# PeterFWS/Structure-PLP-SLAM

Measured on AMD Instinct MI355X. Metric: frames/sec ORB+LSD extract+match, 640x480 TUM-RGBD, 1/2/4/8 GPU, higher is better.
Workload: dtype u8

## Files before the change

### structure-plp-slam_amd/csrc/line_context.hip

```cpp
#include <hip/hip_runtime.h>

#include <algorithm>
#include <cmath>
#include <cstring>
#include <mutex>
#include <vector>

#include "line_device.hpp"
#include "null4.hpp"
#include "seed_sort_model.hpp"
#include "sincos_ziv.hpp"
#include "plp_common.hpp"

using namespace plp;

struct plp_line {
    HostPinned pin;
    int device = 0;
    hipStream_t stream = nullptr;
    hipStream_t idle_stream = nullptr;
    int rows = 0, cols = 0, capB = 0;
    int grow_waves = 0;
    int seed_order = PLP_SEED_ORDER_LIBSTDCXX;
    bool mw_ok = false, seed_sort_ok = false;
    int mw_capB = 0, seed_capB = 0;
    LinePlanes P{};
    LsdParams lp{};
    ResizeExactTab rt{};
    BlurTapsN t11{}, t5{};
    LbdWeightsDev w{};
    DevBuf tabs, blur11, scaled, pix, g2, maxgrad, undef, order, n_order, reg, mw_heap, seed_ent, seed_ws, raw, n_raw, dx, dy, all_kl, all_kl_dir, all_lbd, n_all, status, prof, grow_stats;
    DevBuf l0copy, s_kl, s_lbd, s_fn, s_cnt;
    DevBuf aligned;
    int s_cap = 0;
    int last_B = 0;
    bool last_profiled = false;
    hipStream_t last_stream = nullptr;
    bool profiling = false;
    bool grow_big_ok = false;
    hipEvent_t ev[9] = {};
    double stage_ms[9] = {0, 0, 0, 0, 0, 0, 0, 0, 0};
    long stage_batches = 0;
    std::mutex mu;
};

namespace {

void gaussian_taps(int n, double sigma, int* out) {
    std::vector<double> k(n);
    double sum = 0;
    for (int i = 0; i < n; ++i) { const double x = i - (n - 1) * 0.5; k[i] = std::exp(-0.5 / (sigma * sigma) * x * x); sum += k[i]; }
    double err = 0;
    int acc = 0;
    for (int i = 0; i < n / 2; ++i) {
        const double adj = k[i] / sum * 256.0 + err;
        const int v = (int)std::nearbyint(adj);
        err = adj - v;
        out[i] = out[n - 1 - i] = v;
        acc += v;
    }
    out[n / 2] = 256 - 2 * acc;
}

int floor_d(double v) { int i = (int)v; return i - (i > v); }

void exact_coeffs(int ssize, int dsize, std::vector<int16_t>& ofs, std::vector<int16_t>& c1) {
    const double scale = 1.0 / ((double)dsize / ssize);
    for (int d = 0; d < dsize; ++d) {
        const double val = ((double)d + 0.5) * scale - 0.5;
        const int iv = floor_d(val);
        if (iv >= 0 && ssize > 1) {
            if (iv < ssize - 1) { ofs.push_back((int16_t)iv); c1.push_back((int16_t)std::nearbyint((val - (double)iv) * 256.0)); }
            else { ofs.push_back((int16_t)(ssize - 1)); c1.push_back(-1); }
        } else { ofs.push_back(0); c1.push_back(-2); }
    }
}

plp_status build(plp_line* c, int rows, int cols) {
    if (c->rows == rows && c->cols == cols) return PLP_OK;
    if (rows < 16 || cols < 16 || rows > 16000 || cols > 16000) return set_error(PLP_ERR_INVALID_ARG, "unsupported frame size for the line front-end");
    LinePlanes& P = c->P;
    P.W = cols; P.H = rows;
    P.sw = (int)std::nearbyint(cols * 0.5); P.sh = (int)std::nearbyint(rows * 0.5);
    P.sw_magic = (P.sw >= 2 && P.sw <= 8192) ? (uint32_t)(((1ull << 32) + (uint64_t)P.sw - 1) / (uint64_t)P.sw) : 0u;
// ... 7 lines not shown
    {
        uint32_t g = 0;
        while (g < 600000u && std::sqrt((double)g / 4.0) <= lp.rho) ++g;
        lp.g2_def_min = g;
    }
    lp.density_th = 0.6; lp.scale = 0.5; lp.n_bins = 1024; lp.refine = 1;
    const double LOG_NT = 5 * (std::log10((double)P.sw) + std::log10((double)P.sh)) / 2 + std::log10(11.0);
    lp.min_reg_size = (int)(size_t)(-LOG_NT / std::log10(lp.p));
    lp.min_length = (float)(0.125 * std::min(cols, rows));
    lp.keep_length = 60.f;
    const double sigma = 0.6 / 0.5;
    const unsigned h = (unsigned)std::ceil(sigma * std::sqrt(2 * 3.0 * std::log(10.0)));
    if (h != 5) return set_error(PLP_ERR_UNSUPPORTED, "unexpected LSD kernel size");
    gaussian_taps(11, sigma, c->t11.k);
    for (int i = 0; i < 11; ++i) c->t5.k[i] = 0;
    gaussian_taps(5, 1.0, c->t5.k);
    {
        double u = (7 * 3 - 1) / 2, sg = (7 * 2 + 1) / 2, inv = -1 / (2 * sg * sg);
        for (int i = 0; i < 21; ++i) { const double d = i - u; c->w.l[i] = (float)std::exp(d * d * inv); }
        u = (9 * 7 - 1) / 2; sg = u; inv = -1 / (2 * sg * sg);
        for (int i = 0; i < 63; ++i) { const double d = i - u; c->w.g[i] = (float)std::exp(d * d * inv); }
    }
    std::vector<int16_t> xo, xc, yo, yc;
    exact_coeffs(cols, P.sw, xo, xc);
    exact_coeffs(rows, P.sh, yo, yc);
    {
        bool plain = cols == 2 * P.sw && rows == 2 * P.sh;
        for (int i = 0; plain && i < P.sw; ++i) plain = xo[i] == 2 * i && xc[i] == 128;
        for (int i = 0; plain && i < P.sh; ++i) plain = yo[i] == 2 * i && yc[i] == 128;
        P.half_exact = plain ? 1 : 0;
    }
    std::vector<int16_t> blob;
    blob.insert(blob.end(), xo.begin(), xo.end()); blob.insert(blob.end(), xc.begin(), xc.end());
    blob.insert(blob.end(), yo.begin(), yo.end()); blob.insert(blob.end(), yc.begin(), yc.end());
    PLP_HIP(c->tabs.upload(blob.data(), blob.size() * 2, c->stream));
    PLP_HIP(hipStreamSynchronize(c->stream));
    const int16_t* base = (const int16_t*)c->tabs.p;
    c->rt.xo = base; c->rt.xc = base + P.sw; c->rt.yo = base + 2 * P.sw; c->rt.yc = base + 2 * P.sw + P.sh;
    c->rows = rows; c->cols = cols; c->capB = 0; c->mw_capB = 0; c->seed_capB = 0;
    return PLP_OK;
}

plp_status ensure(plp_line* c, int B) {
    LinePlanes& P = c->P;
    const size_t n = (size_t)P.sw * P.sh, nv = (size_t)(P.sw - 1) * (P.sh - 1);
    const int Bmw = std::min(B, kLsdMwMaxFrames);
    if (B > c->capB) {
        if (!P.half_exact) PLP_HIP(c->blur11.reserve((size_t)P.pitch * P.H * B));
        PLP_HIP(c->scaled.reserve((size_t)P.spitch * P.sh * B));
        PLP_HIP(c->pix.reserve(n * sizeof(LsdPix) * B));
        PLP_HIP(c->g2.reserve(n * 4 * B)); PLP_HIP(c->n_order.reserve(4 * (size_t)B)); PLP_HIP(c->maxgrad.reserve(4 * ((n + 255) / 256) * (size_t)B)); PLP_HIP(c->undef.reserve((n + 63) / 64 * 8 * B));
        PLP_HIP(c->order.reserve(nv * 4 * B)); PLP_HIP(c->reg.reserve(std::max(n * (size_t)B, 2 * n * (size_t)Bmw) * 4));
        PLP_HIP(c->raw.reserve(sizeof(float4) * kLineCap * B)); PLP_HIP(c->n_raw.reserve(4 * (size_t)B));
        PLP_HIP(c->dx.reserve(dxy_frame_entries(P.W, P.H) * 4 * B));
        PLP_HIP(c->all_kl.reserve(sizeof(plp_keyline) * kLineCap * B)); PLP_HIP(c->all_kl_dir.reserve(sizeof(float2) * kLineCap * B)); PLP_HIP(c->all_lbd.reserve((size_t)32 * kLineCap * B));
        PLP_HIP(c->n_all.reserve(4 * (size_t)B)); PLP_HIP(c->status.reserve(16)); PLP_HIP(c->prof.reserve(128)); PLP_HIP(c->grow_stats.reserve(16 * (size_t)B));
        P.blur11 = (uint8_t*)c->blur11.p; P.scaled = (uint8_t*)c->scaled.p;
        P.pix = (LsdPix*)c->pix.p; P.g2 = (uint32_t*)c->g2.p; P.n_order = (int32_t*)c->n_order.p;
        P.blockmax = (uint32_t*)c->maxgrad.p; P.undef = (unsigned long long*)c->undef.p;
        P.order = (uint32_t*)c->order.p; P.reg = (uint32_t*)c->reg.p; P.raw = (float4*)c->raw.p; P.n_raw = (int32_t*)c->n_raw.p;
        P.dxy = (short2*)c->dx.p; P.all_kl = (plp_keyline*)c->all_kl.p; P.all_kl_dir = (float2*)c->all_kl_dir.p; P.all_lbd = (uint8_t*)c->all_lbd.p;
        P.n_all = (int32_t*)c->n_all.p; P.status = (int32_t*)c->status.p; P.prof = (long long*)c->prof.p; P.grow_stats = (int32_t*)c->grow_stats.p;
        c->capB = B;
    }
    P.reg_frame_stride = B <= kLsdMwMaxFrames ? 2 * n : n;
    P.mw_heap_frame_stride = (size_t)(kMwMaxWaves - 1) * kMwHeapBufs * kMwHeap;
    if (c->mw_ok && B <= kLsdMwMaxFrames && B > c->mw_capB) {
        PLP_HIP(c->mw_heap.reserve(P.mw_heap_frame_stride * 4 * (size_t)B));
        c->mw_capB = B;
    }
    P.mw_heap = (B <= c->mw_capB) ? (uint32_t*)c->mw_heap.p : nullptr;
    if (c->seed_order == PLP_SEED_ORDER_LIBSTDCXX && B > c->seed_capB) {
        PLP_HIP(c->seed_ent.reserve(nv * 4 * (size_t)B)); PLP_HIP(c->seed_ws.reserve(seed_sort_ws_entries(nv) * 4 * (size_t)B));
        c->seed_capB = B;
    }
    return PLP_OK;
}

plp_status run(plp_line* c, const uint8_t* d_imgs, int B, int rows, int cols, size_t step, size_t frame_stride, plp_keyline* d_kl,
               uint8_t* d_lbd, double* d_fn, int cap, int32_t* d_counts, hipStream_t st) {
    PLP_HIP(hipSetDevice(c->device));
    if (c->seed_order == PLP_SEED_ORDER_LIBSTDCXX && !c->seed_sort_ok)
        return set_error(PLP_ERR_UNSUPPORTED, "this device refused the dynamic LDS size of the exact seed sort (144 KB per workgroup): select PLP_SEED_ORDER_STABLE with plp_line_set_seed_order");
    PLP_TRY(build(c, rows, cols));
    PLP_TRY(ensure(c, B));
    if (((uintptr_t)d_imgs % 4 == 0) && (step % 4 == 0) && (frame_stride % 4 == 0)) {
        c->P.img = d_imgs; c->P.img_frame_stride = frame_stride; c->P.img_pitch = (int)step;
    } else {
        const size_t fs = (size_t)c->P.pitch * rows;
        PLP_HIP(c->aligned.reserve(fs * B));
        for (int f = 0; f < B; ++f)
            PLP_HIP(hipMemcpy2DAsync((uint8_t*)c->aligned.p + f * fs, c->P.pitch, d_imgs + f * frame_stride, step, cols, rows, hipMemcpyDeviceToDevice, st));
        c->P.img = (const uint8_t*)c->aligned.p; c->P.img_frame_stride = fs; c->P.img_pitch = c->P.pitch;
    }
    PLP_HIP(hipMemsetAsync(c->status.p, 0, 16, st));
    if (c->profiling) PLP_HIP(hipMemsetAsync(c->prof.p, 0, 128, st));
    const bool exact = c->seed_order == PLP_SEED_ORDER_LIBSTDCXX;
    c->lp.seed_exact = exact ? 1 : 0;
    const SeedSortBufs ssb{(uint32_t*)c->seed_ent.p, (uint32_t*)c->seed_ws.p, seed_sort_ws_entries((size_t)(c->P.sw - 1) * (c->P.sh - 1))};
    launch_line_front(st, c->P, c->lp, c->rt, c->t11, c->t5, c->w, d_kl, d_lbd, d_fn, cap, d_counts, B, c->profiling ? c->ev : nullptr,
                      c->grow_waves, exact ? &ssb : nullptr, c->mw_ok);
    PLP_HIP(hipGetLastError());
    if (c->profiling) {
        PLP_HIP(hipEventSynchronize(c->ev[8]));
        for (int i = 0; i < 8; ++i) { float ms = 0; PLP_HIP(hipEventElapsedTime(&ms, c->ev[i], c->ev[i + 1])); c->stage_ms[i] += ms; }
        float tot = 0; PLP_HIP(hipEventElapsedTime(&tot, c->ev[0], c->ev[8])); c->stage_ms[8] += tot;
        ++c->stage_batches;
    }
    c->last_B = B; c->last_stream = st; c->last_profiled = c->profiling;
    return PLP_OK;
}

plp_status batch_status(const int32_t s[4], bool check_cap) {
    if (check_cap && (s[0] & 1)) return set_error(PLP_ERR_CAPACITY, "a frame produced more lines than `cap`; output truncated");
// ... 166 lines not shown
    for (int i = 0; i < 9; ++i) ms9[i] = c->stage_ms[i];
    if (n_batches) *n_batches = c->stage_batches;
    return PLP_OK;
}

plp_status plp_line_scaled_size(const plp_line* c, int32_t* rows, int32_t* cols) {
    if (!c || !rows || !cols || !c->rows) return set_error(PLP_ERR_INVALID_ARG, "no frame processed yet");
    *rows = c->P.sh; *cols = c->P.sw;
    return PLP_OK;
}

plp_status plp_line_debug_read(plp_line* c, plp_line_debug_id what, int32_t frame, void* dst, size_t dst_bytes, int64_t* n_out) {
    if (!c || !dst || !n_out) return set_error(PLP_ERR_INVALID_ARG, "NULL argument");
    std::lock_guard<std::mutex> lk(c->mu);
    if (!c->last_B || frame < 0 || frame >= c->last_B) return set_error(PLP_ERR_INVALID_ARG, "bad frame");
    PLP_HIP(hipSetDevice(c->device));
    PLP_HIP(hipStreamSynchronize(c->last_stream));
    const LinePlanes& P = c->P;
    const size_t n = (size_t)P.sw * P.sh, nv = (size_t)(P.sw - 1) * (P.sh - 1), full = (size_t)P.W * P.H;
    int32_t cnt = 0;
    switch (what) {
        case PLP_LINE_DBG_SCALED:
            if (dst_bytes < n) return set_error(PLP_ERR_CAPACITY, "dst too small");
            PLP_HIP(hipMemcpy2D(dst, P.sw, P.scaled + (size_t)frame * P.spitch * P.sh, P.spitch, P.sw, P.sh, hipMemcpyDeviceToHost));
            *n_out = (int64_t)n; return PLP_OK;
        case PLP_LINE_DBG_ORDER:
            PLP_HIP(hipMemcpy(&cnt, P.n_order + frame, 4, hipMemcpyDeviceToHost));
            if (dst_bytes < (size_t)cnt * 4) return set_error(PLP_ERR_CAPACITY, "dst too small");
            if (cnt) PLP_HIP(hipMemcpy(dst, P.order + (size_t)frame * nv, (size_t)cnt * 4, hipMemcpyDeviceToHost));
            *n_out = cnt; return PLP_OK;
        case PLP_LINE_DBG_RAW:
            PLP_HIP(hipMemcpy(&cnt, P.n_raw + frame, 4, hipMemcpyDeviceToHost));
            if (dst_bytes < (size_t)cnt * 16) return set_error(PLP_ERR_CAPACITY, "dst too small");
            if (cnt) PLP_HIP(hipMemcpy(dst, P.raw + (size_t)frame * kLineCap, (size_t)cnt * 16, hipMemcpyDeviceToHost));
            *n_out = cnt; return PLP_OK;
        case PLP_LINE_DBG_ALL_KL:
        case PLP_LINE_DBG_ALL_LBD: {
            PLP_HIP(hipMemcpy(&cnt, P.n_all + frame, 4, hipMemcpyDeviceToHost));
            const size_t rec = what == PLP_LINE_DBG_ALL_KL ? sizeof(plp_keyline) : 32;
            if (dst_bytes < (size_t)cnt * rec) return set_error(PLP_ERR_CAPACITY, "dst too small");
            const uint8_t* src = what == PLP_LINE_DBG_ALL_KL ? (const uint8_t*)(P.all_kl + (size_t)frame * kLineCap) : P.all_lbd + (size_t)frame * kLineCap * 32;
            if (cnt) PLP_HIP(hipMemcpy(dst, src, (size_t)cnt * rec, hipMemcpyDeviceToHost));
            *n_out = cnt; return PLP_OK;
        }
        case PLP_LINE_DBG_GROW_STATS:
            if (dst_bytes < 16) return set_error(PLP_ERR_CAPACITY, "dst too small");
            PLP_HIP(hipMemcpy(dst, P.grow_stats + (size_t)frame * 4, 16, hipMemcpyDeviceToHost));
            *n_out = 4; return PLP_OK;
        case PLP_LINE_DBG_SOBEL_DX:
        case PLP_LINE_DBG_SOBEL_DY:
            if (dst_bytes < full * 2) return set_error(PLP_ERR_CAPACITY, "dst too small");
            {
                const size_t ent = dxy_frame_entries(P.W, P.H);
                std::vector<int16_t> both(ent * 2);
                PLP_HIP(hipMemcpy(both.data(), P.dxy + (size_t)frame * ent, ent * 4, hipMemcpyDeviceToHost));
                int16_t* d16 = (int16_t*)dst;
                const int tiles8 = (P.W + 7) / 8;
                for (int y = 0; y < P.H; ++y)
                    for (int x = 0; x < P.W; ++x) d16[(size_t)y * P.W + x] = both[2 * (size_t)dxy_index(x, y, tiles8) + (what == PLP_LINE_DBG_SOBEL_DY ? 1 : 0)];
            }
            *n_out = (int64_t)full; return PLP_OK;
    }
    return set_error(PLP_ERR_INVALID_ARG, "unknown debug id");
}

int32_t plp_model_sincos_host(const float* a, int64_t n, float* c, float* s, uint8_t* proven) {
    int32_t n_proven = 0;
    for (int64_t i = 0; i < n; ++i) { proven[i] = plp::sincos_ziv(a[i], c + i, s + i) ? 1 : 0; n_proven += proven[i]; }
    return n_proven;
}

int32_t plp_model_null_vector4_host(const double* A, int32_t n, double* out_v, int32_t* out_sweeps) {
    if (!A || !out_v || n < 0) return -1;
    for (int32_t i = 0; i < n; ++i) {
        int sweeps = 0;
        plp::null_vector4(A + 16 * (size_t)i, out_v + 4 * (size_t)i, &sweeps);
        if (out_sweeps) out_sweeps[i] = sweeps;
    }
    return n;
}

int32_t plp_model_seed_introsort_host(uint32_t* entries, int64_t n, int32_t depth_limit, uint32_t skip_key) {
    if (!entries || n < 0 || n > (int64_t)kLsdMaxScaledPixels) return -1;
    plp::seedsort::introsort_loop_model(entries, (int)n, depth_limit, skip_key);
    return 0;
}

plp_status plp_seed_introsort_debug(int32_t device, uint32_t* entries, int64_t n, int32_t depth_limit, uint32_t skip_key, int32_t variant, int32_t* n_live) {
    if (!entries || n < 0 || n > (int64_t)kLsdMaxScaledPixels) return set_error(PLP_ERR_INVALID_ARG, "bad entries");
    int nd = 0;
    if (hipGetDeviceCount(&nd) != hipSuccess || nd == 0) return set_error(PLP_ERR_NO_DEVICE, "no HIP device visible");
    PLP_HIP(hipSetDevice(device));
    PLP_HIP(seed_sort_configure());
    if (depth_limit < 0) { int lg = 0; while ((2ll << lg) <= n) ++lg; depth_limit = 2 * lg; }
    DevBuf ent, ws, st;
    const int copies = std::max(1, std::min(4096, getenv("PLP_SEED_SORT_DBG_COPIES") ? atoi(getenv("PLP_SEED_SORT_DBG_COPIES")) : 1));
    PLP_HIP(ent.reserve((size_t)std::max<int64_t>(n, 1) * 4 * copies)); PLP_HIP(ws.reserve(seed_sort_ws_entries((size_t)n) * 4 * copies)); PLP_HIP(st.reserve(16));
    for (int k = 0; k < copies; ++k) PLP_HIP(hipMemcpy((uint32_t*)ent.p + (size_t)k * n, entries, (size_t)n * 4, hipMemcpyHostToDevice));
    PLP_HIP(hipMemset(st.p, 0, 16));
    DevBuf dbg;
    const char* dflag = getenv("PLP_SEED_SORT_DBG");
    if (dflag) { PLP_HIP(dbg.reserve(4 * (2 + 6 * 4000 + 48))); PLP_HIP(hipMemset(dbg.p, 0, 4 * (2 + 6 * 4000 + 48))); int f = atoi(dflag); PLP_HIP(hipMemcpy(dbg.p, &f, 4, hipMemcpyHostToDevice)); }
    launch_seed_sort_debug(nullptr, (uint32_t*)ent.p, (int)n, depth_limit, skip_key, (uint32_t*)ws.p, (int32_t*)st.p, dflag ? (int*)dbg.p : nullptr, variant, copies);
    PLP_HIP(hipGetLastError());
    PLP_HIP(hipDeviceSynchronize());
    int32_t s = 0;
    PLP_HIP(hipMemcpy(&s, st.p, 4, hipMemcpyDeviceToHost));
    PLP_HIP(hipMemcpy(entries, ent.p, (size_t)n * 4, hipMemcpyDeviceToHost));
// ... 12 lines not shown
```

### structure-plp-slam_amd/csrc/line_device.hpp

```cpp
#pragma once
#include <hip/hip_runtime.h>
#include <stdint.h>

#include "../../include/plp_front.h"

namespace plp {

constexpr int kMwHeap = 16384;
constexpr int kMwHeapBufs = 2;
constexpr int kMwMaxWaves = 8;
constexpr int kLsdMwMaxFrames = 256;
constexpr int kLineCap = 2048;
constexpr double kLsdNotDef = -1024.0;
constexpr int kLsdSeedPixBits = 20;
constexpr uint32_t kLsdSeedPixMask = (1u << kLsdSeedPixBits) - 1u;
constexpr size_t kLsdGrowLdsBytes = 66560;
constexpr size_t kLsdMaxScaledPixels = (kLsdGrowLdsBytes / 4 - 256) * 32 - 31;
static_assert(kLsdMaxScaledPixels <= (size_t)kLsdSeedPixMask + 1, "seed packing of k_lsd_order must hold every admitted pixel index");
static_assert(kLsdSeedPixBits + 10 <= 32, "10 bits of gradient bin above the pixel field");

struct alignas(16) LsdPix { float deg; uint32_t g2; float2 cs; };
__device__ __forceinline__ double pix_ang(const LsdPix& p) { return (double)p.deg * (3.14159265358979323846 / 180); }
__device__ __forceinline__ double pix_mod(const LsdPix& p) { return sqrt((double)p.g2 / 4.0); }

struct LinePlanes {
    int W, H;
    int sw, sh;
    uint32_t sw_magic;
    int pitch, spitch;
    const uint8_t* img; size_t img_frame_stride; int img_pitch;
    uint8_t* blur11;
    uint8_t* scaled;
    LsdPix* pix;
    uint32_t* g2;
    uint32_t* blockmax;
    unsigned long long* undef;
    uint32_t* order;
    int32_t* n_order;
    uint32_t* reg; size_t reg_frame_stride;
    uint32_t* mw_heap; size_t mw_heap_frame_stride;
    float4* raw; int32_t* n_raw;
    short2* dxy;
    plp_keyline* all_kl; uint8_t* all_lbd; int32_t* n_all;
    float2* all_kl_dir;
    int32_t* status;
    int half_exact;
    int32_t* grow_stats;
    long long* prof;
};

__host__ __device__ inline size_t dxy_frame_entries(int W, int H) { return (size_t)((W + 7) / 8) * ((H + 3) / 4) * 32; }
__host__ __device__ inline int dxy_index(int x, int y, int tiles_x) { return (((y >> 2) * tiles_x + (x >> 3)) << 5) + ((y & 3) << 3) + (x & 7); }

struct LsdParams {
    double prec, p, rho, density_th, scale;
    int n_bins, refine, min_reg_size;
    float min_length;
    float keep_length;
    float c_pass, c_fail;
    uint32_t g2_def_min;
    int seed_exact;
};
constexpr double kLsdAngleBand = 3.5e-4;
constexpr double kLsdBandMinPrec = 0.01, kLsdBandMaxPrec = 1.5;

struct ResizeExactTab { const int16_t *xo, *xc, *yo, *yc; };
struct BlurTapsN { int k[11]; };
struct LbdWeightsDev { float g[63], l[21]; };

struct SeedSortBufs { uint32_t* ent; uint32_t* ws; size_t ws_stride; };
size_t seed_sort_ws_entries(size_t nv);
hipError_t seed_sort_configure();
void launch_seed_order_exact(hipStream_t st, const LinePlanes& P, const LsdParams& lp, int B, uint32_t* ent, uint32_t* ws, size_t ws_stride);
void launch_seed_sort_debug(hipStream_t st, uint32_t* ent, int n, int depth, uint32_t skip_key, uint32_t* ws, int32_t* status, int* dbg, int variant, int copies = 1);
hipError_t grow_mw_configure();
hipError_t grow_configure();

void launch_line_front(hipStream_t st, const LinePlanes& P, const LsdParams& lp, const ResizeExactTab& rt, const BlurTapsN& t11,
                       const BlurTapsN& t5, const LbdWeightsDev& w, plp_keyline* out_kl, uint8_t* out_lbd, double* out_fn, int cap,
                       int32_t* out_counts, int B, hipEvent_t* ev, int grow_waves, const SeedSortBufs* seed_exact, bool mw_ok);

}
```

### structure-plp-slam_amd/csrc/line_kernels.hip

```cpp
#include <hip/hip_runtime.h>
#include <stdint.h>

#include <algorithm>
#include <cstdlib>

#include "blur_tile.hpp"
#include "plp_barrier.hpp"
#include "line_device.hpp"
#include "plp_common.hpp"
#include "sincos_ziv.hpp"
#include "xcd_map.hpp"

namespace plp {

struct TileDiv { uint32_t gx_magic, tiles_x_magic; };
static inline TileDiv tile_div(int tiles, int tiles_x, int B) { return TileDiv{plp_div_magic((uint32_t)tiles, (uint64_t)tiles * B), plp_div_magic((uint32_t)tiles_x, (uint64_t)tiles)}; }

__device__ __forceinline__ int reflect101_l(int p, int len) {
    if (len == 1) return 0;
    while (p < 0 || p >= len) p = p < 0 ? -p : 2 * (len - 1) - p;
    return p;
}

__device__ __forceinline__ float fast_atan2_deg_l(float y, float x) {
// ... 1369 lines not shown
        run += __popcll(bal);
    }
    if (lane == 0) P.n_all[b] = run;
}

constexpr int kSobelTW = 120, kSobelTH = 30;
static_assert(sizeof(BlurTileLds<2>::in) >= kBlurTH * (kBlurTW / 4) * 4, "the blurred tile must fit the input rows it replaces");
__global__ __launch_bounds__(256) __attribute__((amdgpu_waves_per_eu(8, 8))) void k_blur_sobel(const uint8_t* __restrict__ src, size_t src_fs, int src_pitch,
                                                                                            short2* __restrict__ dxy, int w, int h, BlurTapsN taps, TileDiv td) {
    __shared__ __attribute__((aligned(16))) BlurTileLds<2> Sb;
    uint32_t* const bt = reinterpret_cast<uint32_t*>(Sb.in);
    const int tiles_x = (w + kSobelTW - 1) / kSobelTW;
    unsigned t, f;
    xcd_frame_major(t, f, td.gx_magic);
    const int trow = (int)plp_div(t, (unsigned)tiles_x, td.tiles_x_magic);
    const int bx0 = ((int)t - trow * tiles_x) * kSobelTW - 4, by0 = trow * kSobelTH - 1;
    blur_tile_core<2>(Sb, src + (size_t)f * src_fs, src_pitch, w, h, bx0, by0, taps.k, [&](int r0, int c4, const uint32_t (&rows)[kBlurRS]) {
#pragma unroll
        for (int rr = 0; rr < kBlurRS; ++rr) bt[(r0 + rr) * (kBlurTW / 4) + c4 / 4] = rows[rr];
    });
    wg_barrier();
    short2* out_frame = dxy + (size_t)f * dxy_frame_entries(w, h);
    const int tiles8 = (w + 7) / 8;
    for (int i = threadIdx.x; i < (kSobelTW / 4) * (kSobelTH / 2); i += 256) {
        const int cgp = i % (kSobelTW / 4), rp = i / (kSobelTW / 4);
        const int x = bx0 + 4 + 4 * cgp, y = by0 + 1 + 2 * rp;
        if (x >= w || y >= h) continue;
        const int cd = 1 + cgp;
        int d[4][4], sm[4][4];
#pragma unroll
        for (int r = 0; r < 4; ++r) {
            const uint32_t* q = &bt[(2 * rp + r) * (kBlurTW / 4) + cd];
            const uint32_t A = q[-1], Bv = q[0], Cv = q[1];
            const int p[6] = {(int)(A >> 24), (int)(Bv & 255u), (int)((Bv >> 8) & 255u), (int)((Bv >> 16) & 255u), (int)(Bv >> 24), (int)(Cv & 255u)};
#pragma unroll
            for (int k = 0; k < 4; ++k) { d[r][k] = p[k + 2] - p[k]; sm[r][k] = p[k] + 2 * p[k + 1] + p[k + 2]; }
        }
#pragma unroll
        for (int j = 0; j < 2; ++j) {
            if (y + j >= h) continue;
            uint32_t out[4];
#pragma unroll
            for (int k = 0; k < 4; ++k)
                out[k] = ((uint32_t)(d[j][k] + 2 * d[j + 1][k] + d[j + 2][k]) & 0xffffu) | ((uint32_t)(sm[j + 2][k] - sm[j][k]) << 16);
            *reinterpret_cast<uint4*>(out_frame + dxy_index(x, y + j, tiles8)) = make_uint4(out[0], out[1], out[2], out[3]);
        }
    }
}

__constant__ int c_comb[32][2] = {{0, 1}, {0, 2}, {0, 3}, {0, 4}, {0, 5}, {0, 6}, {1, 2}, {1, 3}, {1, 4}, {1, 5}, {1, 6},
                                  {2, 3}, {2, 4}, {2, 5}, {2, 6}, {2, 7}, {2, 8}, {3, 4}, {3, 5}, {3, 6}, {3, 7}, {3, 8},
                                  {4, 5}, {4, 6}, {4, 7}, {4, 8}, {5, 6}, {5, 7}, {5, 8}, {6, 7}, {6, 8}, {7, 8}};

constexpr int kLbdU = 8;
__global__ __launch_bounds__(256) void k_lbd(LinePlanes P, LbdWeightsDev W) {
    __shared__ float s_row[4][63][8];
    __shared__ float s_des[4][72], s_des2[4][72], s_norm[4][4];
    const int lane = threadIdx.x & 63, wv = __builtin_amdgcn_readfirstlane((int)(threadIdx.x >> 6)), b = blockIdx.y;
    const int n_lines = P.n_all[b];
    for (int li = blockIdx.x * 4 + wv; li < n_lines; li += gridDim.x * 4) {
    const plp_keyline kl = P.all_kl[(size_t)b * kLineCap + li];
    const short2* dxyImg = P.dxy + (size_t)b * dxy_frame_entries(P.W, P.H);
    const int tiles8 = (P.W + 7) / 8;
    const short imageWidth = (short)(P.W - 1), imageHeight = (short)(P.H - 1);
    const short lengthOfLSP = (short)kl.numOfPixels;
    const short halfWidth = (short)((lengthOfLSP - 1) / 2), halfHeight = 31;
    const float midX = (float)(0.5 * (double)__fadd_rn(kl.sPointInOctaveX, kl.ePointInOctaveX));
    const float midY = (float)(0.5 * (double)__fadd_rn(kl.sPointInOctaveY, kl.ePointInOctaveY));
    const float2 dir = P.all_kl_dir[(size_t)b * kLineCap + li];
    const float dL0 = dir.x, dL1 = dir.y;
    const float dO0 = -dL1, dO1 = dL0;
    if (lane < 63) {
        float sCorX0 = __fadd_rn(__fadd_rn(__fmul_rn(-dL0, (float)halfWidth), __fmul_rn(dL1, (float)halfHeight)), midX);
        float sCorY0 = __fadd_rn(__fsub_rn(__fmul_rn(-dL1, (float)halfWidth), __fmul_rn(dL0, (float)halfHeight)), midY);
        for (int r = 0; r < lane; ++r) { sCorX0 = __fsub_rn(sCorX0, dL1); sCorY0 = __fadd_rn(sCorY0, dL0); }
        float sCorX = sCorX0, sCorY = sCorY0;
        float pgdL = 0, ngdL = 0, pgdO = 0, ngdO = 0;
        for (int w0 = 0; w0 < lengthOfLSP; w0 += kLbdU) {
            int off[kLbdU];
#pragma unroll
            for (int u = 0; u < kLbdU; ++u) {
                short t = (short)roundf(sCorX);
                const short xCor = (t < 0) ? 0 : (t > imageWidth) ? imageWidth : t;
                t = (short)roundf(sCorY);
                const short yCor = (t < 0) ? 0 : (t > imageHeight) ? imageHeight : t;
                off[u] = dxy_index(xCor, yCor, tiles8);
                sCorX = __fadd_rn(sCorX, dL0);
                sCorY = __fadd_rn(sCorY, dL1);
            }
            short2 vxy[kLbdU];
#pragma unroll
            for (int u = 0; u < kLbdU; ++u) vxy[u] = dxyImg[off[u]];
#pragma unroll
            for (int u = 0; u < kLbdU; ++u) {
                if (w0 + u < lengthOfLSP) {
                    const float fx = (float)vxy[u].x, fy = (float)vxy[u].y;
                    const float gDL = __fadd_rn(__fmul_rn(fx, dL0), __fmul_rn(fy, dL1));
                    const float gDO = __fadd_rn(__fmul_rn(fx, dO0), __fmul_rn(fy, dO1));
                    if (gDL > 0) pgdL = __fadd_rn(pgdL, gDL); else ngdL = __fsub_rn(ngdL, gDL);
                    if (gDO > 0) pgdO = __fadd_rn(pgdO, gDO); else ngdO = __fsub_rn(ngdO, gDO);
                }
            }
        }
        const float cg = W.g[lane];
        pgdL = __fmul_rn(cg, pgdL); ngdL = __fmul_rn(cg, ngdL); pgdO = __fmul_rn(cg, pgdO); ngdO = __fmul_rn(cg, ngdO);
        float* r = s_row[wv][lane];
        r[0] = pgdL; r[1] = ngdL; r[2] = __fmul_rn(pgdL, pgdL); r[3] = __fmul_rn(ngdL, ngdL);
        r[4] = pgdO; r[5] = ngdO; r[6] = __fmul_rn(pgdO, pgdO); r[7] = __fmul_rn(ngdO, ngdO);
    }
    __builtin_amdgcn_fence(__ATOMIC_RELEASE, "workgroup");
    __builtin_amdgcn_wave_barrier();
    for (int item = lane; item < 72; item += 64) {
        const int band = item >> 3, comp = item & 7;
        const bool sq = (comp == 2 || comp == 3 || comp == 6 || comp == 7);
        float acc = 0;
        for (int hID = max(0, (band - 1) * 7); hID < min(63, (band + 2) * 7); ++hID) {
            const int rb = hID / 7;
            const float c = rb == band ? W.l[hID % 7 + 7] : (rb == band + 1 ? W.l[hID % 7 + 14] : W.l[hID % 7]);
            const float v = s_row[wv][hID][comp];
            acc = sq ? __fadd_rn(acc, __fmul_rn(__fmul_rn(c, c), v)) : __fadd_rn(acc, __fmul_rn(c, v));
        }
        s_des[wv][item] = acc;
    }
    __builtin_amdgcn_fence(__ATOMIC_RELEASE, "workgroup");
    __builtin_amdgcn_wave_barrier();
    float* des = s_des2[wv];
    auto wave_sync = [] { __builtin_amdgcn_fence(__ATOMIC_ACQ_REL, "workgroup"); __builtin_amdgcn_wave_barrier(); };
    if (lane < 36) {
        const int band = lane >> 2, k = lane & 3;
        const float invN = (band == 0 || band == 8) ? (float)(1.0 / (7 * 2.0)) : (float)(1.0 / (7 * 3.0));
        const float* sb = &s_des[wv][band * 8];
        const int mi = (k < 2) ? k : k + 2, qi = mi + 2;
        const float temp = __fmul_rn(sb[mi], invN);
        des[band * 8 + k] = temp;
        des[band * 8 + 4 + k] = sqrtf(__fsub_rn(__fmul_rn(sb[qi], invN), __fmul_rn(temp, temp)));
    }
    wave_sync();
    if (lane == 0) {
        float tempM = 0, tempS = 0;
        for (int band = 0; band < 9; ++band) {
            const float* v = des + 8 * band;
            for (int k = 0; k < 4; ++k) tempM = __fadd_rn(tempM, __fmul_rn(v[k], v[k]));
            for (int k = 4; k < 8; ++k) tempS = __fadd_rn(tempS, __fmul_rn(v[k], v[k]));
        }
        s_norm[wv][0] = __fdiv_rn(1.0f, sqrtf(tempM));
        s_norm[wv][1] = __fdiv_rn(1.0f, sqrtf(tempS));
    }
    wave_sync();
    for (int i = lane; i < 72; i += 64) {
        float v = __fmul_rn(des[i], s_norm[wv][(i >> 2) & 1]);
        if ((double)v > 0.4) v = (float)0.4;
        des[i] = v;
    }
    wave_sync();
    if (lane == 0) {
        float temp = 0;
        for (int i = 0; i < 72; ++i) temp = __fadd_rn(temp, __fmul_rn(des[i], des[i]));
        s_norm[wv][2] = __fdiv_rn(1.0f, sqrtf(temp));
    }
    wave_sync();
    for (int i = lane; i < 72; i += 64) des[i] = __fmul_rn(des[i], s_norm[wv][2]);
    wave_sync();
    if (lane < 32) {
        const float* f1 = des + 8 * c_comb[lane][0];
        const float* f2 = des + 8 * c_comb[lane][1];
        unsigned r = 0;
        for (int i = 0; i < 8; ++i) r += (f1[i] > f2[i]) ? (1u << i) : 0u;
        P.all_lbd[((size_t)b * kLineCap + li) * 32 + lane] = (uint8_t)r;
    }
    __builtin_amdgcn_fence(__ATOMIC_ACQ_REL, "workgroup");
    __builtin_amdgcn_wave_barrier();
    }
}

__global__ __launch_bounds__(64) void k_line_finalize(LinePlanes P, LsdParams lp, plp_keyline* __restrict__ out_kl,
                                                      uint8_t* __restrict__ out_lbd, double* __restrict__ out_fn, int cap,
                                                      int32_t* __restrict__ out_counts) {
    const int b = blockIdx.x, lane = threadIdx.x;
    const int n = P.n_all[b];
    int run = 0;
    for (int base = 0; base < n; base += 64) {
        const int i = base + lane;
        plp_keyline kl{};
        bool keep = false;
        if (i < n) { kl = P.all_kl[(size_t)b * kLineCap + i]; keep = kl.octave == 0 && kl.lineLength >= lp.keep_length; }
        const unsigned long long bal = __ballot(keep);
        const int o = run + __popcll(bal & ((1ull << lane) - 1ull));
        if (keep && o < cap) {
            out_kl[(size_t)b * cap + o] = kl;
            const uint4* s = reinterpret_cast<const uint4*>(P.all_lbd + ((size_t)b * kLineCap + i) * 32);
            uint4* d = reinterpret_cast<uint4*>(out_lbd + ((size_t)b * cap + o) * 32);
            d[0] = s[0]; d[1] = s[1];
            const double sx = kl.startPointX, sy = kl.startPointY, ex = kl.endPointX, ey = kl.endPointY;
            const double a = sy * 1.0 - 1.0 * ey, bb = 1.0 * ex - sx * 1.0, c = sx * ey - sy * ex;
            const double nrm = sqrt(a * a + bb * bb);
            double* f = out_fn + ((size_t)b * cap + o) * 3;
            f[0] = a / nrm; f[1] = bb / nrm; f[2] = c / nrm;
        }
        run += __popcll(bal);
    }
    if (lane == 0) {
        out_counts[b] = min(run, cap);
        if (run > cap) atomicOr(P.status, 1);
    }
}

void launch_line_front(hipStream_t st, const LinePlanes& P, const LsdParams& lp, const ResizeExactTab& rt, const BlurTapsN& t11,
                       const BlurTapsN& t5, const LbdWeightsDev& w, plp_keyline* out_kl, uint8_t* out_lbd, double* out_fn, int cap,
                       int32_t* out_counts, int B, hipEvent_t* ev, int grow_waves, const SeedSortBufs* seed_exact, bool mw_ok) {
    auto mark = [&](int i) { if (ev) (void)hipEventRecord(ev[i], st); };
    const bool sobel_first = !ev;
    const size_t plane_fs = (size_t)P.pitch * P.H, splane_fs = (size_t)P.spitch * P.sh;
    const int tiles = ((P.W + 127) / 128) * ((P.H + kBlurTH - 1) / kBlurTH);
    const int sobel_tiles = ((P.W + kSobelTW - 1) / kSobelTW) * ((P.H + kSobelTH - 1) / kSobelTH);
    const TileDiv blur_td = tile_div(tiles, (P.W + 127) / 128, B), sobel_td = tile_div(sobel_tiles, (P.W + kSobelTW - 1) / kSobelTW, B);
    mark(0);
    if (sobel_first) hipLaunchKernelGGL(k_blur_sobel, dim3(sobel_tiles, B), dim3(256), 0, st, P.img, P.img_frame_stride, P.img_pitch, P.dxy, P.W, P.H, t5, sobel_td);
    if (P.half_exact)
        hipLaunchKernelGGL(k_blur_half, dim3(tiles, B), dim3(256), 0, st, P.img, P.img_frame_stride, P.img_pitch, P.scaled, splane_fs, P.spitch, P.W, P.H, t11, blur_td);
    else {
        hipLaunchKernelGGL(k_blur_plane<5>, dim3(tiles, B), dim3(256), 0, st, P.img, P.img_frame_stride, P.img_pitch, P.blur11, plane_fs,
                           P.pitch, P.W, P.H, t11, blur_td);
        hipLaunchKernelGGL(k_resize_exact, dim3((P.sw + 255) / 256, (P.sh + 3) / 4, B), dim3(64, 4), 0, st, P.blur11, plane_fs, P.pitch,
                           P.scaled, splane_fs, P.spitch, P.sw, P.sh, rt);
    }
    mark(1);
    const int n = P.sw * P.sh;
    hipLaunchKernelGGL(k_lsd_gradient, dim3((n + 255) / 256, B), dim3(256), 0, st, P, lp);
    mark(2);
    if (seed_exact) launch_seed_order_exact(st, P, lp, B, seed_exact->ent, seed_exact->ws, seed_exact->ws_stride);
    else hipLaunchKernelGGL(k_lsd_order, dim3(B), dim3(256), 0, st, P, lp, (n + 255) / 256);
    mark(3);
    constexpr int ring = 256;
    const size_t per_wave = (size_t)((((n + 31) / 32 + 1) & ~1) + ring) * 4;
    const int wpb = (int)std::max<size_t>(1, std::min<size_t>(4, 65536 / per_wave));
    MwLayout L{};
    size_t mw_bytes = 0;
    const int want_waves = grow_waves > 0 ? std::min(grow_waves, kMwMaxWaves) : kMwMaxWaves;
    if (mw_ok && B <= kLsdMwMaxFrames && want_waves >= 2 && P.mw_heap && P.reg_frame_stride >= 2 * (size_t)n) {
        const int nw_al = (((n + 31) / 32 + 1) & ~1), groups_cap = ((P.sw - 1) * (P.sh - 1) + kMwGroup - 1) / kMwGroup + 64 / kMwGroup;
        for (int w = want_waves; w >= 2; --w) {
            const size_t bytes = (size_t)5 * nw_al * 4 + (size_t)w * (nw_al + 256 + kMwAssumed + 2) * 4 + (8 + (4 + 2 * kMwBufs) * kMwMaxWaves) * 4 + ((groups_cap + 15) & ~15) + 16 +
                                 (size_t)(w - 1) * kMwBufs * kMwEntries * sizeof(MwEntry);
            if (bytes <= 160 * 1024) { L.waves = w; L.ring = 256; L.nw_al = nw_al; L.n_groups_cap = groups_cap; L.lookahead = kMwBufs * (w - 1); L.policy = 0; L.prof = ev ? 1 : 0; mw_bytes = bytes; break; }
        }
    }
    if (L.waves >= 2)
        hipLaunchKernelGGL(k_lsd_grow_mw, dim3(B), dim3(64 * L.waves), mw_bytes, st, P, lp, L);
    else
        hipLaunchKernelGGL(k_lsd_grow, dim3((B + wpb - 1) / wpb), dim3(64 * wpb), per_wave * wpb, st, P, lp, B, wpb, ring);
    mark(4);
    hipLaunchKernelGGL(k_keylines, dim3(B), dim3(64), 0, st, P, lp);
    mark(5);
    if (!sobel_first) hipLaunchKernelGGL(k_blur_sobel, dim3(sobel_tiles, B), dim3(256), 0, st, P.img, P.img_frame_stride, P.img_pitch, P.dxy, P.W, P.H, t5, sobel_td);
    mark(6);
    const int lbd_blocks = B >= 64 ? 2 : 16;
    hipLaunchKernelGGL(k_lbd, dim3(lbd_blocks, B), dim3(256), 0, st, P, w);
    mark(7);
    hipLaunchKernelGGL(k_line_finalize, dim3(B), dim3(64), 0, st, P, lp, out_kl, out_lbd, out_fn, cap, out_counts);
    mark(8);
}

hipError_t grow_configure() {
    return hipFuncSetAttribute(reinterpret_cast<const void*>(k_lsd_grow), hipFuncAttributeMaxDynamicSharedMemorySize, (int)kLsdGrowLdsBytes);
}
hipError_t grow_mw_configure() {
    return hipFuncSetAttribute(reinterpret_cast<const void*>(k_lsd_grow_mw), hipFuncAttributeMaxDynamicSharedMemorySize, (int)(160 * 1024));
}

}
```

Baseline: 96090.

## Compute LBD Sobel gradients on the fly from a blurred u8 plane staged in LDS

The full-frame Sobel dx/dy plane (short2 per pixel) is no longer materialized. The pipeline now stores only a 5-tap blurred u8 plane, and k_lbd loads a per-segment window of that plane into LDS with global_load_lds. It then computes the 3x3 Sobel at each sampled pixel using udot4 byte dot-products, which cuts global write and read traffic by about 4x per pixel. The cost is extra per-line window loads, wave-min reductions and border reflection logic. The Sobel debug path now recomputes gradients on demand.

```diff
diff --git a/structure-plp-slam_amd/csrc/line_context.hip b/structure-plp-slam_amd/csrc/line_context.hip
--- a/structure-plp-slam_amd/csrc/line_context.hip
+++ b/structure-plp-slam_amd/csrc/line_context.hip
@@ -29,7 +29,7 @@
     ResizeExactTab rt{};
     BlurTapsN t11{}, t5{};
     LbdWeightsDev w{};
-    DevBuf tabs, blur11, scaled, pix, g2, maxgrad, undef, order, n_order, reg, mw_heap, seed_ent, seed_ws, raw, n_raw, dx, dy, all_kl, all_kl_dir, all_lbd, n_all, status, prof, grow_stats;
+    DevBuf tabs, blur11, scaled, pix, g2, maxgrad, undef, order, n_order, reg, mw_heap, seed_ent, seed_ws, raw, n_raw, blur5, sobel_dbg, all_kl, all_kl_dir, all_lbd, n_all, status, prof, grow_stats;
     DevBuf l0copy, s_kl, s_lbd, s_fn, s_cnt;
     DevBuf aligned;
     int s_cap = 0;
@@ -143,14 +143,14 @@
         PLP_HIP(c->g2.reserve(n * 4 * B)); PLP_HIP(c->n_order.reserve(4 * (size_t)B)); PLP_HIP(c->maxgrad.reserve(4 * ((n + 255) / 256) * (size_t)B)); PLP_HIP(c->undef.reserve((n + 63) / 64 * 8 * B));
         PLP_HIP(c->order.reserve(nv * 4 * B)); PLP_HIP(c->reg.reserve(std::max(n * (size_t)B, 2 * n * (size_t)Bmw) * 4));
         PLP_HIP(c->raw.reserve(sizeof(float4) * kLineCap * B)); PLP_HIP(c->n_raw.reserve(4 * (size_t)B));
-        PLP_HIP(c->dx.reserve(dxy_frame_entries(P.W, P.H) * 4 * B));
+        PLP_HIP(c->blur5.reserve((size_t)P.pitch * P.H * B));
         PLP_HIP(c->all_kl.reserve(sizeof(plp_keyline) * kLineCap * B)); PLP_HIP(c->all_kl_dir.reserve(sizeof(float2) * kLineCap * B)); PLP_HIP(c->all_lbd.reserve((size_t)32 * kLineCap * B));
         PLP_HIP(c->n_all.reserve(4 * (size_t)B)); PLP_HIP(c->status.reserve(16)); PLP_HIP(c->prof.reserve(128)); PLP_HIP(c->grow_stats.reserve(16 * (size_t)B));
         P.blur11 = (uint8_t*)c->blur11.p; P.scaled = (uint8_t*)c->scaled.p;
         P.pix = (LsdPix*)c->pix.p; P.g2 = (uint32_t*)c->g2.p; P.n_order = (int32_t*)c->n_order.p;
         P.blockmax = (uint32_t*)c->maxgrad.p; P.undef = (unsigned long long*)c->undef.p;
         P.order = (uint32_t*)c->order.p; P.reg = (uint32_t*)c->reg.p; P.raw = (float4*)c->raw.p; P.n_raw = (int32_t*)c->n_raw.p;
-        P.dxy = (short2*)c->dx.p; P.all_kl = (plp_keyline*)c->all_kl.p; P.all_kl_dir = (float2*)c->all_kl_dir.p; P.all_lbd = (uint8_t*)c->all_lbd.p;
+        P.blur5 = (uint8_t*)c->blur5.p; P.all_kl = (plp_keyline*)c->all_kl.p; P.all_kl_dir = (float2*)c->all_kl_dir.p; P.all_lbd = (uint8_t*)c->all_lbd.p;
         P.n_all = (int32_t*)c->n_all.p; P.status = (int32_t*)c->status.p; P.prof = (long long*)c->prof.p; P.grow_stats = (int32_t*)c->grow_stats.p;
         c->capB = B;
     }
@@ -423,8 +423,12 @@
             if (dst_bytes < full * 2) return set_error(PLP_ERR_CAPACITY, "dst too small");
             {
                 const size_t ent = dxy_frame_entries(P.W, P.H);
+                PLP_HIP(c->sobel_dbg.reserve(ent * 4));
+                launch_sobel_debug(c->last_stream, P, c->t5, frame, (short2*)c->sobel_dbg.p);
+                PLP_HIP(hipGetLastError());
+                PLP_HIP(hipStreamSynchronize(c->last_stream));
                 std::vector<int16_t> both(ent * 2);
-                PLP_HIP(hipMemcpy(both.data(), P.dxy + (size_t)frame * ent, ent * 4, hipMemcpyDeviceToHost));
+                PLP_HIP(hipMemcpy(both.data(), c->sobel_dbg.p, ent * 4, hipMemcpyDeviceToHost));
                 int16_t* d16 = (int16_t*)dst;
                 const int tiles8 = (P.W + 7) / 8;
                 for (int y = 0; y < P.H; ++y)
diff --git a/structure-plp-slam_amd/csrc/line_device.hpp b/structure-plp-slam_amd/csrc/line_device.hpp
--- a/structure-plp-slam_amd/csrc/line_device.hpp
+++ b/structure-plp-slam_amd/csrc/line_device.hpp
@@ -40,7 +40,7 @@
     uint32_t* reg; size_t reg_frame_stride;
     uint32_t* mw_heap; size_t mw_heap_frame_stride;
     float4* raw; int32_t* n_raw;
-    short2* dxy;
+    uint8_t* blur5;
     plp_keyline* all_kl; uint8_t* all_lbd; int32_t* n_all;
     float2* all_kl_dir;
     int32_t* status;
@@ -79,5 +79,6 @@
 void launch_line_front(hipStream_t st, const LinePlanes& P, const LsdParams& lp, const ResizeExactTab& rt, const BlurTapsN& t11,
                        const BlurTapsN& t5, const LbdWeightsDev& w, plp_keyline* out_kl, uint8_t* out_lbd, double* out_fn, int cap,
                        int32_t* out_counts, int B, hipEvent_t* ev, int grow_waves, const SeedSortBufs* seed_exact, bool mw_ok);
+void launch_sobel_debug(hipStream_t st, const LinePlanes& P, const BlurTapsN& t5, int frame, short2* dxy);
 
 }
diff --git a/structure-plp-slam_amd/csrc/line_kernels.hip b/structure-plp-slam_amd/csrc/line_kernels.hip
--- a/structure-plp-slam_amd/csrc/line_kernels.hip
+++ b/structure-plp-slam_amd/csrc/line_kernels.hip
@@ -1445,16 +1445,29 @@
                                   {2, 3}, {2, 4}, {2, 5}, {2, 6}, {2, 7}, {2, 8}, {3, 4}, {3, 5}, {3, 6}, {3, 7}, {3, 8},
                                   {4, 5}, {4, 6}, {4, 7}, {4, 8}, {5, 6}, {5, 7}, {5, 8}, {6, 7}, {6, 8}, {7, 8}};
 
-constexpr int kLbdU = 8;
+constexpr int kLbdSeg = 32;
+constexpr int kLbdU = 2;
+constexpr int kLbdWinDw = 19, kLbdWinRows = 73;
+constexpr int kLbdWinDwords = (kLbdWinRows * kLbdWinDw + 63) / 64 * 64;
+static_assert(kLbdWinDw % 2 == 1, "odd dword pitch: consecutive window rows on different LDS banks");
+static_assert(kLbdWinDwords * 4 >= 63 * 8 * 4, "the row sums of a line reuse its window");
+
+__device__ __forceinline__ int lbd_wave_min(int a, int b) {
+    return min(min(__builtin_amdgcn_readlane(a, 0), __builtin_amdgcn_readlane(a, 62)), min(__builtin_amdgcn_readlane(b, 0), __builtin_amdgcn_readlane(b, 62)));
+}
+
 __global__ __launch_bounds__(256) void k_lbd(LinePlanes P, LbdWeightsDev W) {
-    __shared__ float s_row[4][63][8];
+    __shared__ uint32_t s_win[4][kLbdWinDwords];
     __shared__ float s_des[4][72], s_des2[4][72], s_norm[4][4];
     const int lane = threadIdx.x & 63, wv = __builtin_amdgcn_readfirstlane((int)(threadIdx.x >> 6)), b = blockIdx.y;
+    auto wave_sync = [] { __builtin_amdgcn_fence(__ATOMIC_ACQ_REL, "workgroup"); __builtin_amdgcn_wave_barrier(); };
+    uint32_t* const win32 = s_win[wv];
+    uint8_t* const win = reinterpret_cast<uint8_t*>(s_win[wv]);
+    float (*const s_row)[8] = reinterpret_cast<float (*)[8]>(s_win[wv]);
+    const uint8_t* const blurImg = P.blur5 + (size_t)b * ((size_t)P.pitch * P.H);
     const int n_lines = P.n_all[b];
     for (int li = blockIdx.x * 4 + wv; li < n_lines; li += gridDim.x * 4) {
     const plp_keyline kl = P.all_kl[(size_t)b * kLineCap + li];
-    const short2* dxyImg = P.dxy + (size_t)b * dxy_frame_entries(P.W, P.H);
-    const int tiles8 = (P.W + 7) / 8;
     const short imageWidth = (short)(P.W - 1), imageHeight = (short)(P.H - 1);
     const short lengthOfLSP = (short)kl.numOfPixels;
     const short halfWidth = (short)((lengthOfLSP - 1) / 2), halfHeight = 31;
@@ -1463,41 +1476,99 @@
     const float2 dir = P.all_kl_dir[(size_t)b * kLineCap + li];
     const float dL0 = dir.x, dL1 = dir.y;
     const float dO0 = -dL1, dO1 = dL0;
+    auto coord = [](float v, short hi) -> int {
+        const short t = (short)roundf(v);
+        return (t < 0) ? 0 : (t > hi) ? hi : t;
+    };
+    float sCorX = __fadd_rn(__fadd_rn(__fmul_rn(-dL0, (float)halfWidth), __fmul_rn(dL1, (float)halfHeight)), midX);
+    float sCorY = __fadd_rn(__fsub_rn(__fmul_rn(-dL1, (float)halfWidth), __fmul_rn(dL0, (float)halfHeight)), midY);
+    for (int r = 0; r < min(lane, 62); ++r) { sCorX = __fsub_rn(sCorX, dL1); sCorY = __fadd_rn(sCorY, dL0); }
+    float pgdL = 0, ngdL = 0, pgdO = 0, ngdO = 0;
+    const int xlast = (P.W - 1) & ~3;
+    for (int w0 = 0; w0 < lengthOfLSP;) {
+        int n = min(kLbdSeg, lengthOfLSP - w0);
+        int x0, x1, y0, xa, ndw, nrows;
+        float lastX, lastY;
+        for (;;) {
+            lastX = sCorX; lastY = sCorY;
+            for (int u = 1; u < n; ++u) { lastX = __fadd_rn(lastX, dL0); lastY = __fadd_rn(lastY, dL1); }
+            const int fx = coord(sCorX, imageWidth), fy = coord(sCorY, imageHeight), lx = coord(lastX, imageWidth), ly = coord(lastY, imageHeight);
+            x0 = lbd_wave_min(fx, lx); x1 = -lbd_wave_min(-fx, -lx);
+            y0 = lbd_wave_min(fy, ly);
+            const int y1 = -lbd_wave_min(-fy, -ly);
+            xa = (x0 - 1) & ~3;
+            ndw = ((x1 + 1 - xa) >> 2) + 1;
+            nrows = y1 - y0 + 3;
+            if ((ndw <= kLbdWinDw && nrows <= kLbdWinRows) || n == 1) break;
+            n >>= 1;
+        }
+        ndw = min(ndw, kLbdWinDw); nrows = min(nrows, kLbdWinRows);
+        wave_sync();
+        const int pdw = ndw | 1, pitch = 4 * pdw;
+        const int total = nrows * pdw;
+        const uint32_t pdw_magic = (65536u + (uint32_t)pdw - 1u) / (uint32_t)pdw;
+        for (int i0 = 0; i0 < total; i0 += 64) {
+            const int i = min(i0 + lane, total - 1);
+            const int r = (int)(((uint32_t)i * pdw_magic) >> 16), d = i - r * pdw;
+            int y = y0 - 1 + r;
+            y = y < 0 ? -y : y;
+            y = y >= P.H ? 2 * (P.H - 1) - y : y;
+            const int x = min(max(xa + 4 * d, 0), xlast);
+            __builtin_amdgcn_global_load_lds(reinterpret_cast<const uint32_t*>(blurImg + (uint32_t)(y * P.pitch + x)), win32 + i0, 4, 0, 0);
+        }
+        asm volatile("s_waitcnt vmcnt(0)" ::: "memory");
+        wave_sync();
+        const bool ring_l = x0 == 0, ring_r = x1 == P.W - 1 && P.W - xa < pitch;
+        if (ring_l || ring_r) {
+            for (int r = lane; r < nrows; r += 64) {
+                uint8_t* row = win + r * pitch;
+                if (ring_l) row[-1 - xa] = row[1 - xa];
+                if (ring_r) row[P.W - xa] = row[P.W - 2 - xa];
+            }
+            wave_sync();
+        }
+        const int koff = y0 * pitch + xa + 1;
+        float cx = sCorX, cy = sCorY;
+        for (int c = 0; c < n; c += kLbdU) {
+            int off[kLbdU];
+#pragma unroll
+            for (int u = 0; u < kLbdU; ++u) {
+                const int o = coord(cy, imageHeight) * pitch + coord(cx, imageWidth) - koff;
+                off[u] = (c + u < n) ? o : 0;
+                cx = __fadd_rn(cx, dL0);
+                cy = __fadd_rn(cy, dL1);
+            }
+            int gx[kLbdU], gy[kLbdU];
+#pragma unroll
+            for (int u = 0; u < kLbdU; ++u) {
+                const uint32_t* q = win32 + (off[u] >> 2);
+                const uint32_t sh = (uint32_t)off[u] & 3u;
+                const uint32_t ra = __builtin_amdgcn_alignbyte(q[1], q[0], sh), rb = __builtin_amdgcn_alignbyte(q[pdw + 1], q[pdw], sh);
+                const uint32_t rc = __builtin_amdgcn_alignbyte(q[2 * pdw + 1], q[2 * pdw], sh);
+                const uint32_t right = __builtin_amdgcn_udot4(ra, 0x00010000u, __builtin_amdgcn_udot4(rb, 0x00020000u, __builtin_amdgcn_udot4(rc, 0x00010000u, 0u, false), false), false);
+                const uint32_t left = __builtin_amdgcn_udot4(ra, 0x00000001u, __builtin_amdgcn_udot4(rb, 0x00000002u, __builtin_amdgcn_udot4(rc, 0x00000001u, 0u, false), false), false);
+                gx[u] = (int)right - (int)left;
+                gy[u] = (int)__builtin_amdgcn_udot4(rc, 0x00010201u, 0u, false) - (int)__builtin_amdgcn_udot4(ra, 0x00010201u, 0u, false);
+            }
+#pragma unroll
+            for (int u = 0; u < kLbdU; ++u) {
+                const bool live = c + u < n;
+                const float fx = live ? (float)(short)gx[u] : 0.f, fy = live ? (float)(short)gy[u] : 0.f;
+                const float gDL = __fadd_rn(__fmul_rn(fx, dL0), __fmul_rn(fy, dL1));
+                const float gDO = __fadd_rn(__fmul_rn(fx, dO0), __fmul_rn(fy, dO1));
+                const float pL = __fadd_rn(pgdL, gDL), nL = __fsub_rn(ngdL, gDL), pO = __fadd_rn(pgdO, gDO), nO = __fsub_rn(ngdO, gDO);
+                pgdL = gDL > 0 ? pL : pgdL; ngdL = gDL > 0 ? ngdL : nL;
+                pgdO = gDO > 0 ? pO : pgdO; ngdO = gDO > 0 ? ngdO : nO;
+            }
+        }
+        sCorX = __fadd_rn(lastX, dL0); sCorY = __fadd_rn(lastY, dL1);
+        w0 += n;
+    }
+    wave_sync();
     if (lane < 63) {
-        float sCorX0 = __fadd_rn(__fadd_rn(__fmul_rn(-dL0, (float)halfWidth), __fmul_rn(dL1, (float)halfHeight)), midX);
-        float sCorY0 = __fadd_rn(__fsub_rn(__fmul_rn(-dL1, (float)halfWidth), __fmul_rn(dL0, (float)halfHeight)), midY);
-        for (int r = 0; r < lane; ++r) { sCorX0 = __fsub_rn(sCorX0, dL1); sCorY0 = __fadd_rn(sCorY0, dL0); }
-        float sCorX = sCorX0, sCorY = sCorY0;
-        float pgdL = 0, ngdL = 0, pgdO = 0, ngdO = 0;
-        for (int w0 = 0; w0 < lengthOfLSP; w0 += kLbdU) {
-            int off[kLbdU];
-#pragma unroll
-            for (int u = 0; u < kLbdU; ++u) {
-                short t = (short)roundf(sCorX);
-                const short xCor = (t < 0) ? 0 : (t > imageWidth) ? imageWidth : t;
-                t = (short)roundf(sCorY);
-                const short yCor = (t < 0) ? 0 : (t > imageHeight) ? imageHeight : t;
-                off[u] = dxy_index(xCor, yCor, tiles8);
-                sCorX = __fadd_rn(sCorX, dL0);
-                sCorY = __fadd_rn(sCorY, dL1);
-            }
-            short2 vxy[kLbdU];
-#pragma unroll
-            for (int u = 0; u < kLbdU; ++u) vxy[u] = dxyImg[off[u]];
-#pragma unroll
-            for (int u = 0; u < kLbdU; ++u) {
-                if (w0 + u < lengthOfLSP) {
-                    const float fx = (float)vxy[u].x, fy = (float)vxy[u].y;
-                    const float gDL = __fadd_rn(__fmul_rn(fx, dL0), __fmul_rn(fy, dL1));
-                    const float gDO = __fadd_rn(__fmul_rn(fx, dO0), __fmul_rn(fy, dO1));
-                    if (gDL > 0) pgdL = __fadd_rn(pgdL, gDL); else ngdL = __fsub_rn(ngdL, gDL);
-                    if (gDO > 0) pgdO = __fadd_rn(pgdO, gDO); else ngdO = __fsub_rn(ngdO, gDO);
-                }
-            }
-        }
         const float cg = W.g[lane];
         pgdL = __fmul_rn(cg, pgdL); ngdL = __fmul_rn(cg, ngdL); pgdO = __fmul_rn(cg, pgdO); ngdO = __fmul_rn(cg, ngdO);
-        float* r = s_row[wv][lane];
+        float* r = s_row[lane];
         r[0] = pgdL; r[1] = ngdL; r[2] = __fmul_rn(pgdL, pgdL); r[3] = __fmul_rn(ngdL, ngdL);
         r[4] = pgdO; r[5] = ngdO; r[6] = __fmul_rn(pgdO, pgdO); r[7] = __fmul_rn(ngdO, ngdO);
     }
@@ -1510,7 +1581,7 @@
         for (int hID = max(0, (band - 1) * 7); hID < min(63, (band + 2) * 7); ++hID) {
             const int rb = hID / 7;
             const float c = rb == band ? W.l[hID % 7 + 7] : (rb == band + 1 ? W.l[hID % 7 + 14] : W.l[hID % 7]);
-            const float v = s_row[wv][hID][comp];
+            const float v = s_row[hID][comp];
             acc = sq ? __fadd_rn(acc, __fmul_rn(__fmul_rn(c, c), v)) : __fadd_rn(acc, __fmul_rn(c, v));
         }
         s_des[wv][item] = acc;
@@ -1518,7 +1589,6 @@
     __builtin_amdgcn_fence(__ATOMIC_RELEASE, "workgroup");
     __builtin_amdgcn_wave_barrier();
     float* des = s_des2[wv];
-    auto wave_sync = [] { __builtin_amdgcn_fence(__ATOMIC_ACQ_REL, "workgroup"); __builtin_amdgcn_wave_barrier(); };
     if (lane < 36) {
         const int band = lane >> 2, k = lane & 3;
         const float invN = (band == 0 || band == 8) ? (float)(1.0 / (7 * 2.0)) : (float)(1.0 / (7 * 3.0));
@@ -1602,13 +1672,12 @@
                        const BlurTapsN& t5, const LbdWeightsDev& w, plp_keyline* out_kl, uint8_t* out_lbd, double* out_fn, int cap,
                        int32_t* out_counts, int B, hipEvent_t* ev, int grow_waves, const SeedSortBufs* seed_exact, bool mw_ok) {
     auto mark = [&](int i) { if (ev) (void)hipEventRecord(ev[i], st); };
-    const bool sobel_first = !ev;
+    const bool blur5_first = !ev;
     const size_t plane_fs = (size_t)P.pitch * P.H, splane_fs = (size_t)P.spitch * P.sh;
     const int tiles = ((P.W + 127) / 128) * ((P.H + kBlurTH - 1) / kBlurTH);
-    const int sobel_tiles = ((P.W + kSobelTW - 1) / kSobelTW) * ((P.H + kSobelTH - 1) / kSobelTH);
-    const TileDiv blur_td = tile_div(tiles, (P.W + 127) / 128, B), sobel_td = tile_div(sobel_tiles, (P.W + kSobelTW - 1) / kSobelTW, B);
+    const TileDiv blur_td = tile_div(tiles, (P.W + 127) / 128, B);
     mark(0);
-    if (sobel_first) hipLaunchKernelGGL(k_blur_sobel, dim3(sobel_tiles, B), dim3(256), 0, st, P.img, P.img_frame_stride, P.img_pitch, P.dxy, P.W, P.H, t5, sobel_td);
+    if (blur5_first) hipLaunchKernelGGL(k_blur_plane<2>, dim3(tiles, B), dim3(256), 0, st, P.img, P.img_frame_stride, P.img_pitch, P.blur5, plane_fs, P.pitch, P.W, P.H, t5, blur_td);
     if (P.half_exact)
         hipLaunchKernelGGL(k_blur_half, dim3(tiles, B), dim3(256), 0, st, P.img, P.img_frame_stride, P.img_pitch, P.scaled, splane_fs, P.spitch, P.W, P.H, t11, blur_td);
     else {
@@ -1645,7 +1714,7 @@
     mark(4);
     hipLaunchKernelGGL(k_keylines, dim3(B), dim3(64), 0, st, P, lp);
     mark(5);
-    if (!sobel_first) hipLaunchKernelGGL(k_blur_sobel, dim3(sobel_tiles, B), dim3(256), 0, st, P.img, P.img_frame_stride, P.img_pitch, P.dxy, P.W, P.H, t5, sobel_td);
+    if (!blur5_first) hipLaunchKernelGGL(k_blur_plane<2>, dim3(tiles, B), dim3(256), 0, st, P.img, P.img_frame_stride, P.img_pitch, P.blur5, plane_fs, P.pitch, P.W, P.H, t5, blur_td);
     mark(6);
     const int lbd_blocks = B >= 64 ? 2 : 16;
     hipLaunchKernelGGL(k_lbd, dim3(lbd_blocks, B), dim3(256), 0, st, P, w);
@@ -1654,6 +1723,12 @@
     mark(8);
 }
 
+void launch_sobel_debug(hipStream_t st, const LinePlanes& P, const BlurTapsN& t5, int frame, short2* dxy) {
+    const int tiles_x = (P.W + kSobelTW - 1) / kSobelTW, sobel_tiles = tiles_x * ((P.H + kSobelTH - 1) / kSobelTH);
+    hipLaunchKernelGGL(k_blur_sobel, dim3(sobel_tiles, 1), dim3(256), 0, st, P.img + (size_t)frame * P.img_frame_stride, P.img_frame_stride, P.img_pitch, dxy,
+                       P.W, P.H, t5, tile_div(sobel_tiles, tiles_x, 1));
+}
+
 hipError_t grow_configure() {
     return hipFuncSetAttribute(reinterpret_cast<const void*>(k_lsd_grow), hipFuncAttributeMaxDynamicSharedMemorySize, (int)kLsdGrowLdsBytes);
 }
```

New measurement: 96900, median of 6. About the same (+0.8%).
